# DigITs-AIML/MMNN_STS

Measured on AMD Instinct MI355X. Metric: training volumes/sec/GPU (128^3 T1+T2+preop, batch 2) at 1/2/4/8 MI355X, higher is better.
Workload: dtype f32; 1 GPU; configs[2] --images --preop --survival --blend: MultiModalModel(DenseNet121-3D(in=2), MLP(32), blend) fwd + GradientBlender Cox loss + bwd + grad all-reduce + SGD-Nesterov/OneCycle step, dropout 0.2; micro_batch=2, global_batch=2, tabular=32, parallelism=dp1, allreduce=none

## Files before the change

mmnn_sts_amd/csrc/densenet.hip:

```cpp
#include "densenet.hpp"

#include <string.h>

#include <algorithm>

#include "fprop.hpp"
#include "stem.hpp"
#include "wgrad.hpp"

namespace mmnn {

constexpr size_t KZ_PART_BYTES = (size_t)512 * 4 * 1024 * sizeof(float);
constexpr unsigned KZ_CNT_ENTRIES = 4096;

namespace {
struct Panel { const float* p; unsigned bytes; };
struct LayerBind {
  BnFwd bn1, bn2;
  BnBwd gr_new, gr_t1;
  StatPtr dg1, dg2, s_x;
  View x, g;
  View x_new, g_new;
  View t1, dz2;
};
// ... 361 lines not shown
      p.timer_ev.push_back(a); p.timer_ev.push_back(b);
      p.timer_tag.push_back(0);
    }
    p.timer_tag[p.timer_used / 2] = kind * MAX_BLOCKS + (block >= 0 && block < MAX_BLOCKS ? block : 0);
    on = hipEventRecord(p.timer_ev[p.timer_used], s) == hipSuccess;
  }
  ~ScopedTimer() {
    if (!on) return;
    (void)hipEventRecord(p.timer_ev[p.timer_used + 1], s);
    p.timer_used += 2;
  }
};
}

int plan_set_timer(Plan& p, int kind, int block) {
  MMNN_REQUIRE(kind >= -1 && kind < T_COUNT, "set_timer: unknown kernel class %d", kind);
  p.timer_mask = kind < 0 ? ~1u : (kind == T_NONE ? 0u : 1u << kind);
  p.timer_block = block; p.timer_used = 0;
  for (int k = 0; k < T_COUNT * MAX_BLOCKS; ++k) { p.timer_ms[k] = 0.0; p.timer_count[k] = 0; }
  return 0;
}

int plan_read_timer(Plan& p, int kind, int block, double* total_ms, long* count) {
  MMNN_REQUIRE(kind >= T_NONE && kind < T_COUNT && block < MAX_BLOCKS, "read_timer: unknown kernel class %d / block %d", kind, block);
  for (size_t i = 0; i + 1 < p.timer_used; i += 2) {
    MMNN_HIP(hipEventSynchronize(p.timer_ev[i + 1]));
    float ms = 0.f;
    MMNN_HIP(hipEventElapsedTime(&ms, p.timer_ev[i], p.timer_ev[i + 1]));
    const int k = p.timer_tag[i / 2];
    p.timer_ms[k] += ms; p.timer_count[k] += 1;
  }
  p.timer_used = 0;
  double ms = 0.0; long n = 0;
  for (int k = 1; k < T_COUNT; ++k)
    for (int b = 0; b < MAX_BLOCKS; ++b)
      if ((kind == T_NONE || kind == k) && (block < 0 || block == b)) { ms += p.timer_ms[k * MAX_BLOCKS + b]; n += p.timer_count[k * MAX_BLOCKS + b]; }
  if (total_ms) *total_ms = ms;
  if (count) *count = n;
  return 0;
}

int plan_set_option(Plan& p, const char* name, long value) {
  const std::string s(name ? name : "");
  if (s == "single_stream") return 0;
  if (s == "trace_buffer") { p.trace_base = reinterpret_cast<unsigned long long*>(value); p.trace_seq = 0; return 0; }
  if (s == "trace_slots") { p.trace_slots = (int)value; return 0; }
  if (s == "params_version") { p.params_version = value; return 0; }
  if (s == "no_kz") { p.no_kz = value != 0; return 0; }
  if (s == "conv1_dgrad_resident") {
    MMNN_REQUIRE(value >= 0 && value <= 2, "set_option: conv1_dgrad_resident is 0, 1 or 2");
    p.conv1_dgrad_resident = (int)value;
    return 0;
  }
  set_error("set_option: unknown option '%s'", s.c_str());
  return 1;
}
static DropCfg dropcfg(const Plan& p, uint64_t seed, int layer, int training) {
  DropCfg d; memset(&d, 0, sizeof(d));
  d.seed = seed; d.layer = layer; d.p = training ? p.cfg.dropout_p : 0.f;
  return d;
}

int plan_forward(Plan& p, const float* params, float* run, const float* x, char* ws, float* out, int training, uint64_t seed,
                 hipStream_t stream) {
  MMNN_REQUIRE(params && run && x && ws && out, "forward: null buffer");
  MMNN_REQUIRE(((uintptr_t)ws & 255) == 0 && ((uintptr_t)params & 15) == 0 && ((uintptr_t)x & 15) == 0, "forward: buffers must be 256/16-byte aligned");
  const NetCfg& c = p.cfg;
  const int nb = c.nblocks, N = p.N;
  if (!p.host_jobs) {
    MMNN_HIP(hipHostMalloc(&p.host_jobs, p.host_jobs_bytes, hipHostMallocDefault));
    memset(p.host_jobs, 0, p.host_jobs_bytes);
  }
  if (p.tab_params != params || p.tab_run != run || p.tab_ws != ws) {
    if (p.tab_ws != nullptr) MMNN_HIP(hipStreamSynchronize(stream));
    build_tables(p, params, run, ws);
    MMNN_HIP(hipMemcpyAsync(ws + p.o_jobs_run, p.host_jobs, p.host_jobs_bytes, hipMemcpyHostToDevice, stream));
  }
  p.trace_seq = 0;
  if (training) MMNN_HIP(hipMemsetAsync(ws + p.o_fstat, 0, p.fstat_bytes, stream));
  MMNN_HIP(hipMemsetAsync(ws + p.o_kz_cnt, 0, KZ_CNT_ENTRIES * sizeof(unsigned), stream));
  int rc = 0;
  if (p.params_version == 0 || p.params_version != p.packed_version || p.packed_params != params || p.packed_ws != ws) {
    rc = launch_pack(reinterpret_cast<const PackJob*>(ws + p.o_jobs_pack), p.n_pack_jobs, p.max_pack, stream);
    if (rc) return rc;
    p.packed_version = p.params_version; p.packed_params = params; p.packed_ws = ws;
    ++p.pack_launches;
  }

  {
    const NormSite n0 = norm0(p);
    StemConvArgs a; memset(&a, 0, sizeof(a));
    a.N = N; a.Cin = c.in_channels; a.D = p.D; a.H = p.H; a.W = p.W; a.Do = p.D0; a.Ho = p.H0; a.Wo = p.W0; a.M = c.init_features;
    a.x = x; a.wp = fptr(ws, p.o_pk_conv0); a.out = fptr(ws, p.o_conv0);
    a.st_out = stats(ws, n0, 0, training);
    { ScopedTimer t(p, T_STEM_CONV, -1, stream); rc = launch_stem_conv(a, stream); }
    if (rc) return rc;
    const View X = concat(p, ws, 0);
    StemPoolArgs q; memset(&q, 0, sizeof(q));
    q.N = N; q.C = c.init_features; q.Di = p.D0; q.Hi = p.H0; q.Wi = p.W0; q.Do = p.Db[0]; q.Ho = p.Hb[0]; q.Wo = p.Wb[0];
    q.x = fptr(ws, p.o_conv0);
    q.bn = bnfwd(p, ws, params, run, n0, training);
    q.out = X.p; q.out_ns = X.ns;
    q.idx = reinterpret_cast<unsigned char*>(ws + p.o_idx);
    q.st_out = stats(ws, norm1(p, 0, 0), 0, training);
    if ((rc = launch_stem_pool(q, stream))) return rc;
  }
// ... 33 lines not shown
      q.bn = bnfwd(p, ws, params, run, tr, training);
      q.out = pooled(p, ws, b).p;
      if ((rc = launch_bnrelu_avgpool(q, stream))) return rc;
      FpropArgs a = block_args(p, ws, b + 1);
      a.Cin = p.trans[b].cin; a.M = p.trans[b].cout;
      set_in0(a, pooled(p, ws, b));
      a.w = trans_panel(p, ws, b).p; a.w_ld = a.M;
      set_out(a, concat(p, ws, b + 1));
      a.st_out = stats(ws, norm1(p, b + 1, 0), 0, training);
      prefetch(a, conv1_panel(p, ws, b + 1, 0));
      if ((rc = launch_fprop(a, 1, PRO_NONE, EPI_STORE_STATS, stream))) return rc;
    } else {
      const NormSite n5 = norm5(p);
      BnApplyArgs q; memset(&q, 0, sizeof(q));
      q.N = N; q.C = n5.C; q.V = p.Vb[b];
      q.x = X.p; q.x_ns = X.ns;
      q.bn = bnfwd(p, ws, params, run, n5, training);
      q.out = out;
      if ((rc = launch_bn_apply(q, stream))) return rc;
    }
  }
  if (training) {
    if ((rc = launch_running_stats(reinterpret_cast<const RunStatJob*>(ws + p.o_jobs_run), p.n_run_jobs, c.momentum,
                                   p.nbt_count == p.n_run_jobs ? p.nbt : nullptr, stream))) return rc;
  }
  return 0;
}

static LayerBind layer_bind(const Plan& p, const float* params, float* run, char* ws, int b, int l) {
  const NormSite n1 = norm1(p, b, l), n2 = norm2(p, b, l);
  LayerBind L; memset(&L, 0, sizeof(L));
  L.bn1 = bnfwd(p, ws, params, run, n1, 1); L.bn2 = bnfwd(p, ws, params, run, n2, 1);
  L.gr_new = bnbwd(p, ws, params, n1, n1.C); L.gr_t1 = bnbwd(p, ws, params, n2);
  L.dg1 = dgsums(ws, n1); L.dg2 = dgsums(ws, n2); L.s_x = sums(ws, n1);
  L.x = concat(p, ws, b); L.g = concat_grad(p, ws, b);
  L.x_new = concat(p, ws, b, n1.C); L.g_new = concat_grad(p, ws, b, n1.C);
  L.t1 = t1(p, ws, b, l); L.dz2 = dz2(p, ws, b, l);
  return L;
}

static void layer_wgrad_args(const Plan& p, const LayerBind& L, char* ws, int b, int l, int layer_id, WgradArgs& w2, WgradArgs& w1) {
  const int cin = p.layers[b][l].cin;
  wgrad_shape(w2, p, b);
  w2.M = p.cfg.growth; w2.Cin = p.mid;
  set_g0(w2, L.g_new); set_g1(w2, L.x_new); w2.gr = L.gr_new;
  w2.drop.layer = layer_id; w2.drop.p = p.cfg.dropout_p;
  set_x(w2, L.t1); w2.bn = L.bn2;
  w2.slab = fptr(ws, p.o_sl_c2[b][l]); w2.slab_stride = conv2_elems(p); w2.nsplit = p.ns_c2[b][l];
  wgrad_shape(w1, p, b);
  w1.M = p.mid; w1.Cin = cin;
  set_g0(w1, L.dz2); set_g1(w1, L.t1); w1.gr = L.gr_t1;
  set_x(w1, L.x); w1.bn = L.bn1;
  w1.slab = fptr(ws, p.o_sl_c1[b][l]); w1.slab_stride = conv1_elems(p, cin); w1.nsplit = p.ns_c1[b][l];
}

static ConsumerBwdArgs consumer_bwd_args(const Plan& p, const float* params, float* run, char* ws, const NormSite& s, int b, int mode, const float* dy) {
  const View X = concat(p, ws, b), G = concat_grad(p, ws, b);
  const StatPtr dg = dgsums(ws, s);
  ConsumerBwdArgs a; memset(&a, 0, sizeof(a));
  a.N = p.N; a.C = s.C; a.D = p.Db[b]; a.H = p.Hb[b]; a.W = p.Wb[b]; a.mode = mode; a.nrep = s.nrep;
  a.dy = dy; a.x = X.p; a.x_ns = X.ns;
  a.bn = bnfwd(p, ws, params, run, s, 1);
  a.g = G.p; a.g_ns = G.ns; a.dbeta = dg.sum; a.dgamma = dg.sq;
  a.s_acc = sums(ws, s);
  return a;
}

int plan_backward(Plan& p, const float* params, const float* x, char* ws, const float* grad_out, float* grad_params, int accumulate,
                  uint64_t seed, hipStream_t stream) {
  return plan_backward_range(p, params, x, ws, grad_out, grad_params, accumulate, seed, p.cfg.nblocks - 1, 0, stream);
}

int plan_block_param_range(const Plan& p, int block, long* begin, long* end) {
  const int nb = p.cfg.nblocks;
  MMNN_REQUIRE(block >= -1 && block < nb && begin && end, "block_param_range: block %d out of range [-1, %d)", block, nb);
  if (block < 0) { *begin = 0; *end = norm1(p, 0, 0).w; return 0; }
  *begin = norm1(p, block, 0).w;
  *end = (block + 1 < nb) ? norm1(p, block + 1, 0).w : p.n_params;
  return 0;
}

int plan_backward_range(Plan& p, const float* params, const float* x, char* ws, const float* grad_out, float* grad_params, int accumulate,
                        uint64_t seed, int hi, int lo, hipStream_t stream) {
  MMNN_REQUIRE(params && x && ws && grad_out && grad_params, "backward: null buffer");
  MMNN_REQUIRE(p.tab_ws == ws && p.tab_params == params, "backward: must follow a training forward on the same buffers");
  const NetCfg& c = p.cfg;
  const int nb = c.nblocks, N = p.N;
  MMNN_REQUIRE(hi >= lo && lo >= 0 && hi < nb, "backward: bad block range [%d, %d] of %d blocks", lo, hi, nb);
  MMNN_REQUIRE(hi == nb - 1 || p.bwd_next == hi, "backward: block range [%d, %d] out of order (expected to continue at block %d)", lo, hi, p.bwd_next);
  float* run = p.tab_run;
  int rc;
  const bool first_call = hi == nb - 1;
  if (first_call) {
    MMNN_HIP(hipMemsetAsync(ws + p.o_bstat, 0, p.bstat_bytes, stream));
    MMNN_HIP(hipMemsetAsync(ws + p.o_kz_cnt, 0, KZ_CNT_ENTRIES * sizeof(unsigned), stream));
  }
  p.bwd_next = lo - 1;
  if (first_call || !p.wg_uploaded) {
    const size_t bytes = sizeof(WgradArgs) * 2 * p.n_layers;
    if (!p.wg_pinned) {
      MMNN_HIP(hipHostMalloc(&p.wg_pinned, bytes, hipHostMallocDefault));
      p.wg_shadow.assign(bytes, 0);
      p.wg_uploaded = false;
    }
    std::vector<WgradArgs> tab(2 * p.n_layers);
    int id = 0;
// ... 24 lines not shown
      int i = j - 1;
      while (i > id0 && wgrad1_channel_width(host_w1[i - 1].Cin, p.Vb[b]) == wgrad1_channel_width(host_w1[j - 1].Cin, p.Vb[b])) --i;
      {
        ScopedTimer t(p, T_CONV1_WGRAD, b, stream);
        rc2 = j - i > 1 ? launch_wgrad_batched(host_w1 + i, dev_w1 + i, j - i, seed, 1, PRO_BNRELU, stream)
                        : launch_wgrad1(host_w1[i], PRO_BNRELU, stream);
      }
      if (rc2) return rc2;
      j = i;
    }
    return 0;
  };
  if (first_call && (rc = launch_consumer_bwd(consumer_bwd_args(p, params, run, ws, norm5(p), nb - 1, 0, grad_out), stream))) return rc;
  int layer_id = 0;
  for (int b = 0; b <= hi; ++b) layer_id += c.block_layers[b];
  for (int b = hi; b >= lo; --b) {
    for (int l = c.block_layers[b] - 1; l >= 0; --l) {
      --layer_id;
      const LayerBind L = layer_bind(p, params, run, ws, b, l);
      const int cin = p.layers[b][l].cin;
      FpropArgs a = block_args(p, ws, b);
      a.Cin = c.growth; a.M = p.mid;
      set_in0(a, L.g_new); set_in1(a, L.x_new); a.gr_in = L.gr_new;
      a.drop_in = dropcfg(p, seed, layer_id, 1);
      set_conv2_weights(a, p, ws, b, l, true); a.w_ld = p.mid;
      set_out(a, L.dz2); set_ex(a, L.t1); a.ebn = L.bn2;
      a.dbeta = L.dg2.sum; a.dgamma = L.dg2.sq;
      prefetch(a, conv1_weights(p, params, b, l));
      { ScopedTimer t(p, T_CONV2_DGRAD, b, stream); rc = launch_fprop(a, 27, PRO_GRAD, EPI_MASK_STORE, stream); }
      if (rc) return rc;
      FpropArgs d = block_args(p, ws, b);
      d.Cin = p.mid; d.M = cin;
      set_in0(d, L.dz2); set_in1(d, L.t1); d.gr_in = L.gr_t1;
      d.w = conv1_weights(p, params, b, l).p; d.w_ld = cin;
      set_out(d, L.g); set_ex(d, L.x); d.ebn = L.bn1;
      d.dbeta = L.dg1.sum; d.dgamma = L.dg1.sq;
      d.s_acc = L.s_x;
      if (l > 0) prefetch(d, conv2_panel(p, ws, b, l - 1, true));
      { ScopedTimer t(p, T_CONV1_DGRAD, b, stream); rc = launch_fprop(d, 1, PRO_GRAD, EPI_MASK_ACCUM, stream); }
      if (rc) return rc;
    }
    if ((rc = block_wgrads(b, layer_id))) return rc;
    const View X = concat(p, ws, b), G = concat_grad(p, ws, b);
    const BnBwd gr = bnbwd(p, ws, params, norm1(p, b, 0));
    if (b > 0) {
      const int pb = b - 1;
      const TransOff& t = p.trans[pb];
      WgradArgs w;
      wgrad_shape(w, p, b);
      w.M = t.cout; w.Cin = t.cin;
      set_g0(w, G); set_g1(w, X); w.gr = gr;
      set_x(w, pooled(p, ws, pb));
      w.slab = fptr(ws, p.o_sl_tr[pb]); w.slab_stride = trans_elems(t); w.nsplit = p.ns_tr[pb];
      if ((rc = launch_wgrad1(w, PRO_NONE, stream))) return rc;
      FpropArgs d = block_args(p, ws, b);
      d.nrep = 0;
      d.Cin = t.cout; d.M = t.cin;
      set_in0(d, G); set_in1(d, X); d.gr_in = gr;
      d.w = params + t.cw; d.w_ld = t.cin;
      set_out(d, pooled_grad(p, ws, pb));
      if ((rc = launch_fprop(d, 1, PRO_GRAD, EPI_STORE, stream))) return rc;
      if ((rc = launch_consumer_bwd(consumer_bwd_args(p, params, run, ws, transition(p, pb), pb, 1, pooled_grad(p, ws, pb).p), stream))) return rc;
    } else {
      const NormSite n0 = norm0(p);
      const StatPtr dg = dgsums(ws, n0);
      StemPoolBwdArgs q; memset(&q, 0, sizeof(q));
      q.N = N; q.C = c.init_features; q.Di = p.D0; q.Hi = p.H0; q.Wi = p.W0; q.Do = p.Db[0]; q.Ho = p.Hb[0]; q.Wo = p.Wb[0];
      q.x = fptr(ws, p.o_conv0);
      q.bn = bnfwd(p, ws, params, run, n0, 1);
      q.g = G.p; q.g_ns = G.ns; q.xp = X.p; q.xp_ns = X.ns;
      q.gr = gr;
      q.idx = reinterpret_cast<const unsigned char*>(ws + p.o_idx);
      q.dz = fptr(ws, p.o_dz0);
      q.dbeta = dg.sum; q.dgamma = dg.sq;
      if ((rc = launch_stem_pool_bwd(q, stream))) return rc;
      StemWgradArgs w; memset(&w, 0, sizeof(w));
      w.N = N; w.Cin = c.in_channels; w.D = p.D; w.H = p.H; w.W = p.W; w.Do = p.D0; w.Ho = p.H0; w.Wo = p.W0; w.M = c.init_features;
      w.x = x; w.dz = fptr(ws, p.o_dz0); w.y = fptr(ws, p.o_conv0);
      w.gr = bnbwd(p, ws, params, n0);
      w.slab = fptr(ws, p.o_sl_conv0); w.slab_stride = (long)c.in_channels * c.init_features * 352; w.nsplit = p.ns_conv0;
      { ScopedTimer t(p, T_STEM_WGRAD, -1, stream); rc = launch_stem_wgrad(w, stream); }
      if (rc) return rc;
    }
  }
  const long stem_count = (long)c.init_features * c.in_channels * 343;
  const GradJob* jobs = reinterpret_cast<const GradJob*>(ws + p.o_jobs_grad);
  const int j0 = lo == 0 ? 0 : p.gj_begin[lo], j1 = p.gj_begin[hi + 1];
  long jmax = lo == 0 ? stem_count : 0;
  for (int b = lo; b <= hi; ++b) jmax = std::max(jmax, p.gj_max[b]);
  return launch_finalize(jobs + j0, j1 - j0, jmax, grad_params, accumulate, stream);
}

int plan_relu_mask(Plan& p, const float* params, char* ws, int kind, int b, int l, unsigned char* out, hipStream_t stream) {
  MMNN_REQUIRE(p.tab_ws == ws && p.tab_params == params, "relu_mask: must follow a training forward on the same buffers");
  const NetCfg& c = p.cfg;
  MMNN_REQUIRE(kind == 0 || (b >= 0 && b < c.nblocks), "relu_mask: bad block %d", b);
  MMNN_REQUIRE(kind != 3 || b < c.nblocks - 1, "relu_mask: block %d has no transition", b);
  MMNN_REQUIRE(kind == 0 || kind == 3 || (l >= 0 && l < c.block_layers[b] && (kind == 1 || kind == 2)), "relu_mask: bad site (%d,%d,%d)", kind, b, l);
  const NormSite s = kind == 0 ? norm0(p) : kind == 1 ? norm1(p, b, l) : kind == 2 ? norm2(p, b, l) : transition(p, b);
  const int V = kind == 0 ? p.D0 * p.H0 * p.W0 : p.Vb[b];
  const View X = kind == 0 ? View{fptr(ws, p.o_conv0), (long)s.C * V, 0} : kind == 2 ? t1(p, ws, b, l) : concat(p, ws, b);
  MaskArgs a; memset(&a, 0, sizeof(a));
  a.out = out; a.N = p.N; a.C = s.C; a.V = V; a.x = X.p; a.x_ns = X.ns;
  a.bn = bnfwd(p, ws, params, p.tab_run, s, 1);
  return launch_relu_mask(a, stream);
}
// ... 41 lines not shown
```

mmnn_sts_amd/csrc/densenet.hpp:

```cpp
#pragma once
#include <string>
#include <vector>

#include "common.hpp"
#include "elementwise.hpp"

namespace mmnn {

constexpr int MAX_BLOCKS = 8;

struct NetCfg {
  int in_channels, init_features, growth, bn_size, nblocks;
  int block_layers[MAX_BLOCKS];
  float eps, momentum, dropout_p;
};

struct LayerOff {
  long n1w, n1b, c1, n2w, n2b, c2;
  long r1m, r1v, r2m, r2v;
  int cin;
};
struct TransOff { long nw, nb, cw; long rm, rv; int cin, cout; };

struct NormSite {
// ... 7 lines not shown
struct View { float* p; long ns; int coff; };

struct Plan {
  NetCfg cfg;
  int N, D, H, W;
  int D0, H0, W0;
  int Db[MAX_BLOCKS], Hb[MAX_BLOCKS], Wb[MAX_BLOCKS], Vb[MAX_BLOCKS];
  int cin_b[MAX_BLOCKS], ctot_b[MAX_BLOCKS];
  int nrep_b[MAX_BLOCKS];
  int mid;
  long p_conv0, p_n0w, p_n0b, r_n0m, r_n0v, p_n5w, p_n5b, r_n5m, r_n5v;
  std::vector<std::vector<LayerOff>> layers;
  std::vector<TransOff> trans;
  long n_params, n_runstats;
  int n_bn;
  size_t ws_bytes;
  size_t o_conv0, o_idx, o_x[MAX_BLOCKS], o_g[MAX_BLOCKS], o_ap[MAX_BLOCKS], o_dz2[MAX_BLOCKS], o_dap, o_dz0;
  std::vector<std::vector<size_t>> o_t1;
  size_t o_fstat, fstat_bytes, o_bstat, bstat_bytes;
  size_t o_st_conv0, o_st_x[MAX_BLOCKS];
  std::vector<std::vector<size_t>> o_st_t1;
  size_t o_s_x[MAX_BLOCKS];
  size_t o_dg_n0, o_dg_n5;
  std::vector<std::vector<size_t>> o_dg_n1, o_dg_n2;
  std::vector<size_t> o_dg_tr;
  size_t o_pk_conv0;
  std::vector<std::vector<size_t>> o_pk_c1, o_pk_c2f, o_pk_c2b;
  std::vector<std::vector<size_t>> o_pk_c2f3, o_pk_c2b3;
  size_t o_x3 = 0, x3_bytes = 0;
  std::vector<size_t> o_pk_tr;
  size_t o_sl_conv0; int ns_conv0;
  std::vector<std::vector<size_t>> o_sl_c1, o_sl_c2;
  std::vector<std::vector<int>> ns_c1, ns_c2;
  std::vector<size_t> o_sl_tr; std::vector<int> ns_tr;
  size_t o_kz_part, o_kz_cnt;
  size_t o_jobs_run, o_jobs_pack, o_jobs_grad;
  int n_layers = 0;
  size_t o_wg_table = 0;
  void* wg_pinned = nullptr; std::vector<char> wg_shadow; bool wg_uploaded = false;
  void* host_jobs = nullptr; size_t host_jobs_bytes = 0;
  const float* tab_params = nullptr; float* tab_run = nullptr; char* tab_ws = nullptr;
  int n_run_jobs = 0, n_pack_jobs = 0, n_grad_jobs = 0; long max_pack = 0, max_grad = 0;
  int gj_begin[MAX_BLOCKS + 1] = {0};
  long gj_max[MAX_BLOCKS] = {0};
  unsigned timer_mask = 0; int timer_block = -1;
  std::vector<hipEvent_t> timer_ev;
  std::vector<int> timer_tag;
  size_t timer_used = 0;
  double timer_ms[16 * MAX_BLOCKS] = {0}; long timer_count[16 * MAX_BLOCKS] = {0};
  long params_version = 0, packed_version = 0; const float* packed_params = nullptr; const char* packed_ws = nullptr;
  long pack_launches = 0;
  long long* nbt = nullptr; int nbt_count = 0;
  int conv1_dgrad_resident = 1;
  bool no_kz = false;
  int bwd_next = -1;
  unsigned long long* trace_base = nullptr; mutable int trace_seq = 0; int trace_slots = 0;
};

enum TimerKind { T_NONE = 0, T_CONV2_FWD = 1, T_CONV2_DGRAD = 2, T_CONV2_WGRAD = 3, T_CONV1_FWD = 4, T_CONV1_DGRAD = 5,
                 T_CONV1_WGRAD = 6, T_STEM_CONV = 7, T_STEM_WGRAD = 8, T_BLOCK_FWD = 9, T_COUNT = 10 };
int plan_set_timer(Plan& p, int kind, int block);
int plan_read_timer(Plan& p, int kind, int block, double* total_ms, long* count);
int plan_set_option(Plan& p, const char* name, long value);

int plan_build(Plan& p, const NetCfg& cfg, int N, int D, int H, int W);
void plan_free(Plan& p);
int plan_forward(Plan& p, const float* params, float* runstats, const float* x, char* ws, float* out, int training,
                 uint64_t seed, hipStream_t stream);
int plan_backward(Plan& p, const float* params, const float* x, char* ws, const float* grad_out, float* grad_params,
                  int accumulate, uint64_t seed, hipStream_t stream);
int plan_backward_range(Plan& p, const float* params, const float* x, char* ws, const float* grad_out, float* grad_params,
                        int accumulate, uint64_t seed, int hi, int lo, hipStream_t stream);
int plan_block_param_range(const Plan& p, int block, long* begin, long* end);
long plan_ws_offset(const Plan& p, const char* name, int i, int j);
int plan_relu_mask(Plan& p, const float* params, char* ws, int kind, int b, int l, unsigned char* out, hipStream_t stream);

}
```

mmnn_sts_amd/csrc/wgrad.hip:

```cpp
#include "wgrad.hpp"

#include <algorithm>

namespace mmnn {

static void wg3_tile(int W, int& TD, int& TH, int& TW) {
  if (W > 16) { TD = 1; TH = 2; TW = 32; }
  else if (W > 8) { TD = 1; TH = 4; TW = 16; }
  else if (W > 4) { TD = 2; TH = 4; TW = 8; }
  else { TD = 4; TH = 4; TW = 4; }
}

static int wg1_wc(int Cin, long V) {
  const int thr = V >= 32768 ? 256 : 97;
  return Cin >= thr ? 8 : 4;
}

int wgrad_pick_splits(int taps, int N, int D, int H, int W, int M, int Cin, int batch) {
  if (batch < 1) batch = 1;
  if (taps == 27) {
    int TD, TH, TW;
    wg3_tile(W, TD, TH, TW);
    const long ntiles = (long)N * cdiv(D, TD) * cdiv(H, TH) * cdiv(W, TW);
    const int cgroups = cdiv(Cin, 32);
    long s = 512 / ((long)cgroups * batch);
    if (s > 64) s = 64;
    if (s > ntiles / 2) s = ntiles / 2;
    return s < 1 ? 1 : (int)s;
  }
  const long V = (long)D * H * W;
  const long nchunks = (long)N * cdiv(V, 64);
  const int wc = wg1_wc(Cin, V);
  constexpr long target = 2048;
  const long groups = (long)cdiv(Cin, 32 * wc) * cdiv(M, 128);
  long s = batch > 1 ? target / batch : target / groups;
  const long slab_cap = ((long)64 << 20) / ((long)M * Cin * 4);
  if (s > slab_cap) s = slab_cap;
  if (s > nchunks / 2) s = nchunks / 2;
  return s < 1 ? 1 : (int)s;
}

int wgrad1_channel_width(int Cin, long V) { return 32 * wg1_wc(Cin, V); }

int wgrad3_launch_batched(const WgradArgs* host, const WgradArgs* dev, int count, uint64_t seed, hipStream_t stream);
int wgrad1_launch(const WgradArgs& a, int pro_x, int wc, hipStream_t s);
int wgrad1_launch_batched(const WgradArgs* host, const WgradArgs* dev, int count, uint64_t seed, int wc, hipStream_t stream);

int launch_wgrad_batched(const WgradArgs* host, const WgradArgs* dev, int count, uint64_t seed, int taps, int pro_x, hipStream_t stream) {
  MMNN_REQUIRE(host && dev && count >= 1 && count <= 65535, "wgrad batch: bad table (count %d)", count);
  MMNN_REQUIRE(pro_x == PRO_BNRELU, "wgrad batch: only the dense-layer kernels (BN+ReLU input prologue) are batched");
  MMNN_REQUIRE(taps == 1 || taps == 27, "wgrad: taps must be 1 or 27");
  const WgradArgs& f = host[0];
  for (int i = 0; i < count; ++i) {
    const WgradArgs& a = host[i];
    MMNN_REQUIRE(a.N == f.N && a.D == f.D && a.H == f.H && a.W == f.W && a.M == f.M, "wgrad batch: layer %d differs in extent", i);
    MMNN_REQUIRE(a.N > 0 && a.D > 0 && a.H > 0 && a.W > 0 && a.Cin > 0 && a.M > 0, "wgrad: non-positive extent");
    MMNN_REQUIRE((long)a.D * a.H * a.W < (1l << 30), "wgrad: volume too large for 32-bit voxel indices");
    MMNN_REQUIRE(taps != 27 || (long)33 * a.D * a.H * a.W < (1l << 31), "wgrad: volume too large for 32-bit element offsets of a 32-channel group");
    MMNN_REQUIRE(a.g0 && a.g1 && a.x && a.slab, "wgrad: null operand");
    MMNN_REQUIRE(a.nsplit >= 1 && a.nsplit <= 65535, "wgrad: bad split count %d", a.nsplit);
    MMNN_REQUIRE(a.slab_stride >= (long)taps * a.M * a.Cin, "wgrad: slab stride too small");
    MMNN_REQUIRE(taps == 27 ? a.M <= 32 : a.M <= 128, "wgrad batch: %d output channels exceed one block row", a.M);
    MMNN_REQUIRE(taps == 27 || wg1_wc(a.Cin, (long)a.D * a.H * a.W) == wg1_wc(f.Cin, (long)f.D * f.H * f.W), "wgrad batch: layer %d needs another channel-group width", i);
  }
  if (taps == 27) return wgrad3_launch_batched(host, dev, count, seed, stream);
  return wgrad1_launch_batched(host, dev, count, seed, wg1_wc(f.Cin, (long)f.D * f.H * f.W), stream);
}

int launch_wgrad1(const WgradArgs& a, int pro_x, hipStream_t stream) {
  MMNN_REQUIRE(a.N > 0 && a.D > 0 && a.H > 0 && a.W > 0 && a.Cin > 0 && a.M > 0, "wgrad: non-positive extent");
  MMNN_REQUIRE((long)a.D * a.H * a.W < (1l << 30), "wgrad: volume too large for 32-bit voxel indices");
  MMNN_REQUIRE(a.g0 && a.g1 && a.x && a.slab, "wgrad: null operand");
  MMNN_REQUIRE(a.nsplit >= 1 && a.nsplit <= 65535, "wgrad: bad split count %d", a.nsplit);
  MMNN_REQUIRE(a.slab_stride >= (long)a.M * a.Cin, "wgrad: slab stride too small");
  MMNN_REQUIRE(pro_x == PRO_BNRELU || pro_x == PRO_NONE, "wgrad: unsupported input prologue %d", pro_x);
  return wgrad1_launch(a, pro_x, wg1_wc(a.Cin, (long)a.D * a.H * a.W), stream);
}

}
```

mmnn_sts_amd/csrc/wgrad.hpp:

```cpp
#pragma once
#include <type_traits>

#include "common.hpp"
#include "wgrad_tile.hpp"

namespace mmnn {

struct WgradArgs {
  int N, D, H, W;
  int M, Cin;
  const float* g0; long g0_ns; int g0_coff;
  const float* g1; long g1_ns; int g1_coff;
  BnBwd gr;
  DropCfg drop;
  const float* x; long x_ns; int x_coff;
  BnFwd bn;
  float* slab; long slab_stride; int nsplit;
  unsigned long long* trace;
};

int launch_wgrad1(const WgradArgs& a, int pro_x, hipStream_t stream);
int launch_wgrad_batched(const WgradArgs* host, const WgradArgs* dev_table, int count, uint64_t seed, int taps, int pro_x, hipStream_t stream);
int wgrad1_channel_width(int Cin, long V);
int wgrad_pick_splits(int taps, int N, int D, int H, int W, int M, int Cin, int batch = 1);

#if defined(__HIPCC__)

#if !defined(MMNN_TRACE_TID)
#define MMNN_TRACE_TID 0
#endif

template <int TD, int TH, int TW>
struct Wg3Cfg {
  static constexpr int VT = TD * TH * TW;
  static constexpr int RS = TW + 2, HS = TH + 2, DS = TD + 2;
  static constexpr int XS = (DS * HS * RS) | 1;
  static constexpr int YS = VT + 1;
  static constexpr int NTHREADS = 8 * 64;
  static_assert(VT == 64, "tile must hold 64 voxels (two per MFMA k-step, 32 steps)");
  static_assert(32 % TW == 0, "tile width must divide 32");
  static constexpr int STAGE = 32 * XS + 32 * YS;
  static size_t smem_bytes() { return sizeof(float) * (2 * STAGE + 3 * 32 + 2 * 32 + 3 * 32); }
};

template <int NTP, int TD, int TH, int TW, class F>
__device__ __forceinline__ void wg3_mfma(f32x16 (&acc)[4], const float* yl, const float* x0, const float* x1, const float* x2, const float* x3, F&& filler) {
  constexpr int RS = Wg3Cfg<TD, TH, TW>::RS, HS = Wg3Cfg<TD, TH, TW>::HS;
  mfma_ksteps<32, 1, NTP>(
      acc, [&](int s, float (&av)[1]) { av[0] = yl[s]; },
      [&](int s, float (&bv)[NTP]) {
        int wx, hy, dz;
        tile_local<TH, TW>(s, wx, hy, dz);
        const int p0 = (dz * HS + hy) * RS + wx;
        bv[0] = x0[p0]; bv[1] = x1[p0]; bv[2] = x2[p0];
        if constexpr (NTP == 4) bv[3] = x3[p0];
      },
      filler);
}

template <int PRO_X, int TD, int TH, int TW>
__device__ __forceinline__ void wgrad3_body(const WgradArgs& a, const int split, const int cg) {
  using C = Wg3Cfg<TD, TH, TW>;
  constexpr int RS = C::RS, HS = C::HS, DS = C::DS, XS = C::XS, YS = C::YS, NTHREADS = C::NTHREADS;
  extern __shared__ __attribute__((aligned(16))) float smem[];
  float* Xs = smem;
  float* Ys = Xs + 32 * XS;
  float* gcoef = smem + 2 * C::STAGE;
  float* xcoef = gcoef + 96;
  float* gbase = xcoef + 64;
  const int tid = threadIdx.x, lane = tid & 63, wave = tid >> 6, half = lane >> 5, l31 = lane & 31;
// ... 216 lines not shown
      const int d = d0 + dz - 1, h = h0 + hy - 1, w = w0 + q - 1;
      const bool ok = c0 + cl < a.Cin && (unsigned)d < (unsigned)a.D && (unsigned)h < (unsigned)a.H && (unsigned)w < (unsigned)a.W;
      const float x = xn[ok ? (long)cl * V + ((long)d * a.H + h) * a.W + w : 0];
      Xs[cl * XS + (dz * HS + hy) * RS + q] = ok ? pro_apply<PRO_X>(xcoef, 32, cl, x, 0.f) : 0.f;
    }
#pragma unroll 4
    for (int it = tid; it < 32 * 64; it += NTHREADS) {
      const int t = it & 63, m = it >> 6;
      int wx, hy, dz;
      tile_local<TH, TW>(t, wx, hy, dz);
      const int d = d0 + dz, h = h0 + hy, w = w0 + wx;
      const bool ok = m < a.M && d < a.D && h < a.H && w < a.W;
      const long g = ok ? (long)m * V + ((long)d * a.H + h) * a.W + w : 0;
      const float o = pro_apply<PRO_GRAD>(gcoef, 32, m, g0n[g], g1n[g]);
      Ys[m * YS + t] = ok ? o : 0.f;
    }
    __syncthreads();
    mfma_tile(0, NoFiller{});
    __syncthreads();
  }
  }
  float* out = a.slab + (long)split * a.slab_stride + c0 + l31;
#pragma unroll
  for (int j = 0; j < 4; ++j)
    if (j < ntap) store_acc_tile(acc[j], out + (long)(tap0 + j) * a.M * a.Cin, a.Cin, 0, a.M, half, c0 + l31 < a.Cin);
}

template <int PRO_X, int TD, int TH, int TW>
__global__ void __launch_bounds__(512) wgrad3_batched_kernel(const WgradArgs* __restrict__ table, const uint64_t seed, const int nsplit,
                                                             const int cgroups, const int ngroups) {
  int z, split, cg;
  if (ngroups > 0) {
    const int lin = blockIdx.x, x = lin & 7, j = lin >> 3;
    const int G = x + 8 * (j / cgroups);
    cg = j % cgroups;
    if (G >= ngroups) return;
    z = G / nsplit; split = G - z * nsplit;
  } else {
    z = blockIdx.z; split = blockIdx.x; cg = blockIdx.y;
  }
  WgradArgs a = table[z];
  if (split >= a.nsplit || cg * 32 >= a.Cin) return;
  a.drop.seed = seed;
  wgrad3_body<PRO_X, TD, TH, TW>(a, split, cg);
}

template <int WC>
struct Wg1Cfg {
  static constexpr int VK = 64, S = VK + 1;
  static constexpr int NTHREADS = WC * 64;
  static size_t smem_bytes() { return sizeof(float) * (128 * S + 32 * WC * S + 3 * 128 + 2 * 32 * WC + 3 * 128); }
};

template <int PRO_X, int WC>
__device__ __forceinline__ void wgrad1_body(const WgradArgs& a, const int split, const int c0, const int m0) {
  using C = Wg1Cfg<WC>;
  constexpr int S = C::S, VK = C::VK, NTHREADS = C::NTHREADS, CB = 32 * WC;
  extern __shared__ __attribute__((aligned(16))) float smem[];
  float* As = smem;
  float* Bs = As + 128 * S;
  float* gcoef = Bs + CB * S;
  float* xcoef = gcoef + 384;
  float* gbase = xcoef + 2 * CB;
  const int tid = threadIdx.x, lane = tid & 63, wave = tid >> 6, half = lane >> 5, l31 = lane & 31;
  const int V = a.D * a.H * a.W;
  const int chunks_per_n = (V + VK - 1) / VK;
  int k_begin, k_end;
  split_range(a.N * chunks_per_n, split, a.nsplit, k_begin, k_end);

  auto coefficients = [&]() {
    for (int c = tid; c < CB; c += NTHREADS) pro_coef_row(xcoef, CB, c, c0 + c, PRO_X == PRO_BNRELU && c0 + c < a.Cin, a.bn);
    for (int m = tid; m < 128; m += NTHREADS) pro_coef_row(gbase, 128, m, m0 + m, m0 + m < a.M, a.gr);
  };
  f32x16 acc[4] = {};
  const float* al = As + l31 * S + 32 * half;
  const float* bl = Bs + (wave * 32 + l31) * S + 32 * half;
  const bool wave_has_channels = c0 + wave * 32 < a.Cin;
  const bool vec = (V & 3) == 0 && ((((uintptr_t)a.x | (uintptr_t)a.g0 | (uintptr_t)a.g1) & 15) == 0);

  auto mfma_chunk = [&]() {
    mfma_ksteps<32, 4, 1>(
        acc,
        [&](int s, float (&av)[4]) {
#pragma unroll
          for (int t = 0; t < 4; ++t) av[t] = al[t * 32 * S + s];
        },
        [&](int s, float (&bv)[1]) { bv[0] = bl[s]; }, NoFiller{});
  };

  if (vec) {
    constexpr int A_ITEMS = 128 * (VK / 4), B_ITEMS = CB * (VK / 4);
    constexpr int A_IT = (A_ITEMS + NTHREADS - 1) / NTHREADS, B_IT = (B_ITEMS + NTHREADS - 1) / NTHREADS;
    f32x4 ga[A_IT], gb[A_IT], xb[B_IT];
    unsigned oka = 0, okb = 0;
    auto load_chunk = [&](int ch) {
      const int n = ch / chunks_per_n, v0 = (ch % chunks_per_n) * VK;
      const gcf xn = (gcf)a.x + (long)n * a.x_ns + (long)(a.x_coff + c0) * V;
      const gcf g0n = (gcf)a.g0 + (long)n * a.g0_ns + (long)(a.g0_coff + m0) * V;
      const gcf g1n = (gcf)a.g1 + (long)n * a.g1_ns + (long)(a.g1_coff + m0) * V;
      oka = okb = 0;
#pragma unroll
      for (int i = 0; i < A_IT; ++i) {
        const int it = tid + i * NTHREADS;
        const int q = it % (VK / 4), m = it / (VK / 4);
        const int v = v0 + 4 * q;
        const bool ok = (it < A_ITEMS) && m0 + m < a.M && v < V;
        const long go = ok ? (long)m * V + v : 0;
        oka |= (ok ? 1u : 0u) << i;
        ga[i] = *reinterpret_cast<const MMNN_GLOBAL f32x4*>(g0n + go);
        gb[i] = *reinterpret_cast<const MMNN_GLOBAL f32x4*>(g1n + go);
      }
#pragma unroll
      for (int i = 0; i < B_IT; ++i) {
        const int it = tid + i * NTHREADS;
        const int q = it % (VK / 4), c = it / (VK / 4);
        const int v = v0 + 4 * q;
        const bool ok = (it < B_ITEMS) && c0 + c < a.Cin && v < V;
        okb |= (ok ? 1u : 0u) << i;
        xb[i] = *reinterpret_cast<const MMNN_GLOBAL f32x4*>(xn + (ok ? (long)c * V + v : 0));
      }
    };
    auto store_chunk = [&]() {
#pragma unroll
      for (int i = 0; i < A_IT; ++i) {
        const int it = tid + i * NTHREADS;
        if (it < A_ITEMS) {
          const int q = it % (VK / 4), m = it / (VK / 4);
          const bool ok = (oka >> i) & 1u;
#pragma unroll
          for (int e = 0; e < 4; ++e) As[m * S + 4 * q + e] = ok ? pro_apply<PRO_GRAD>(gcoef, 128, m, ga[i][e], gb[i][e]) : 0.f;
        }
      }
#pragma unroll
      for (int i = 0; i < B_IT; ++i) {
        const int it = tid + i * NTHREADS;
        if (it < B_ITEMS) {
          const int q = it % (VK / 4), c = it / (VK / 4);
          const bool ok = (okb >> i) & 1u;
#pragma unroll
          for (int e = 0; e < 4; ++e) Bs[c * S + 4 * q + e] = ok ? pro_apply<PRO_X>(xcoef, CB, c, xb[i][e], 0.f) : 0.f;
        }
      }
    };
// ... 13 lines not shown
      pt.lap(1);
      __syncthreads();
      pt.lap(2);
      if (ch + 1 < k_end) load_chunk(ch + 1);
      pt.lap(3);
      if (wave_has_channels) mfma_chunk();
      pt.lap(4);
      __syncthreads();
      pt.lap(5);
    }
    pt.finish(a.trace, split, 1, a.M, a.Cin, k_end - k_begin);
  } else {
  coefficients();
  int cur_n = -1;
  for (int ch = k_begin; ch < k_end; ++ch) {
    const int n = ch / chunks_per_n;
    const int v0 = (ch % chunks_per_n) * VK;
    if (n != cur_n) {
      __syncthreads();
      rescale_rows(gbase, gcoef, 128, m0, n, a.drop, tid, NTHREADS);
      cur_n = n;
      __syncthreads();
    }
    const float* xn = a.x + (long)n * a.x_ns + (long)(a.x_coff + c0) * V;
    const float* g0n = a.g0 + (long)n * a.g0_ns + (long)(a.g0_coff + m0) * V;
    const float* g1n = a.g1 + (long)n * a.g1_ns + (long)(a.g1_coff + m0) * V;
#pragma unroll 2
    for (int it = tid; it < 128 * VK; it += NTHREADS) {
      const int q = it % VK, m = it / VK;
      const int v = v0 + q;
      float o = 0.f;
      if (m0 + m < a.M && v < V) o = pro_apply<PRO_GRAD>(gcoef, 128, m, g0n[(long)m * V + v], g1n[(long)m * V + v]);
      As[m * S + q] = o;
    }
#pragma unroll 2
    for (int it = tid; it < CB * VK; it += NTHREADS) {
      const int q = it % VK, c = it / VK;
      const int v = v0 + q;
      float o = 0.f;
      if (c0 + c < a.Cin && v < V) o = pro_apply<PRO_X>(xcoef, CB, c, xn[(long)c * V + v], 0.f);
      Bs[c * S + q] = o;
    }
    __syncthreads();
    if (wave_has_channels) mfma_chunk();
    __syncthreads();
  }
  }
  const int c = c0 + wave * 32 + l31;
  float* out = a.slab + (long)split * a.slab_stride + c;
#pragma unroll
  for (int t = 0; t < 4; ++t) store_acc_tile(acc[t], out, a.Cin, m0 + t * 32, a.M, half, c < a.Cin);
}

template <int PRO_X, int WC>
__global__ void __launch_bounds__(WC * 64) wgrad1_kernel(const WgradArgs a) {
  wgrad1_body<PRO_X, WC>(a, blockIdx.x, blockIdx.y * (32 * WC), blockIdx.z * 128);
}

template <int PRO_X, int WC>
__global__ void __launch_bounds__(WC * 64) wgrad1_batched_kernel(const WgradArgs* __restrict__ table, const uint64_t seed) {
  const int split = blockIdx.x, cg = blockIdx.y;
  WgradArgs a = table[blockIdx.z];
  if (split >= a.nsplit || cg * (32 * WC) >= a.Cin) return;
  a.drop.seed = seed;
  wgrad1_body<PRO_X, WC>(a, split, cg * (32 * WC), 0);
}

#endif
}
```

mmnn_sts_amd/csrc/wgrad_k1.hip:

```cpp
#include <algorithm>

#include "wgrad.hpp"

namespace mmnn {

template <int PRO_X, int WC>
static int launch1(const WgradArgs& a, hipStream_t stream) {
  using C = Wg1Cfg<WC>;
  constexpr auto kern = wgrad1_kernel<PRO_X, WC>;
  const size_t smem = C::smem_bytes();
  if (int rc = allow_dynamic_lds<kern>(smem)) return rc;
  MMNN_LAUNCH(kern, dim3(a.nsplit, cdiv(a.Cin, 32 * WC), cdiv(a.M, 128)), dim3(C::NTHREADS), smem, stream, a);
  MMNN_HIP(hipGetLastError());
  return 0;
}

template <int PRO_X, int WC>
static int launch1_batched(const WgradArgs* host, const WgradArgs* dev, int count, uint64_t seed, hipStream_t stream) {
  using C = Wg1Cfg<WC>;
  constexpr auto kern = wgrad1_batched_kernel<PRO_X, WC>;
  const size_t smem = C::smem_bytes();
  if (int rc = allow_dynamic_lds<kern>(smem)) return rc;
  int gx = 1, gy = 1;
  for (int i = 0; i < count; ++i) { gx = std::max(gx, host[i].nsplit); gy = std::max(gy, cdiv(host[i].Cin, 32 * WC)); }
  MMNN_LAUNCH(kern, dim3(gx, gy, count), dim3(C::NTHREADS), smem, stream, dev, seed);
  MMNN_HIP(hipGetLastError());
  return 0;
}

int wgrad1_launch(const WgradArgs& a, int pro_x, int wc, hipStream_t s) {
  if (pro_x == PRO_BNRELU) return wc == 8 ? launch1<PRO_BNRELU, 8>(a, s) : launch1<PRO_BNRELU, 4>(a, s);
  return wc == 8 ? launch1<PRO_NONE, 8>(a, s) : launch1<PRO_NONE, 4>(a, s);
}

int wgrad1_launch_batched(const WgradArgs* host, const WgradArgs* dev, int count, uint64_t seed, int wc, hipStream_t stream) {
  return wc == 8 ? launch1_batched<PRO_BNRELU, 8>(host, dev, count, seed, stream) : launch1_batched<PRO_BNRELU, 4>(host, dev, count, seed, stream);
}

}
```

Baseline: 264.8 volumes/s (whole job; 1 volume = 1 patient = stacked T1+T2 2x128^3 + 32 tabular).

## Software-pipeline the 1x1 wgrad tile loop, interleaving global loads with MFMA k-steps

Adds a pipelined variant of the 1x1 weight-gradient kernel that splits each 32-wide chunk into two 16-step halves. It issues the global loads and LDS stores for the next half inside the MFMA k-steps using sched_group_barrier, and precomputes per-row prologue coefficients into registers. It also sets launch bounds to allow two blocks per CU for the pipelined kernel and turns it on by default behind a new option. The aim is to hide global-memory latency behind the matrix math, at the cost of more registers and more complex scheduling.

New measurement: 266.3 volumes/s (whole job; 1 volume = 1 patient = stacked T1+T2 2x128^3 + 32 tabular), median of 6. Within noise of the previous version (+0.6%).

```diff
diff --git a/mmnn_sts_amd/csrc/densenet.hip b/mmnn_sts_amd/csrc/densenet.hip
--- a/mmnn_sts_amd/csrc/densenet.hip
+++ b/mmnn_sts_amd/csrc/densenet.hip
@@ -437,6 +437,11 @@
     p.conv1_dgrad_resident = (int)value;
     return 0;
   }
+  if (s == "wgrad1_pipelined") {
+    MMNN_REQUIRE(value == 0 || value == 1, "set_option: wgrad1_pipelined is 0 or 1");
+    p.wgrad1_pipelined = (int)value;
+    return 0;
+  }
   set_error("set_option: unknown option '%s'", s.c_str());
   return 1;
 }
@@ -576,6 +581,7 @@
   set_g0(w1, L.dz2); set_g1(w1, L.t1); w1.gr = L.gr_t1;
   set_x(w1, L.x); w1.bn = L.bn1;
   w1.slab = fptr(ws, p.o_sl_c1[b][l]); w1.slab_stride = conv1_elems(p, cin); w1.nsplit = p.ns_c1[b][l];
+  w1.pipelined = p.wgrad1_pipelined;
 }
 
 static ConsumerBwdArgs consumer_bwd_args(const Plan& p, const float* params, float* run, char* ws, const NormSite& s, int b, int mode, const float* dy) {
@@ -706,6 +712,7 @@
       set_g0(w, G); set_g1(w, X); w.gr = gr;
       set_x(w, pooled(p, ws, pb));
       w.slab = fptr(ws, p.o_sl_tr[pb]); w.slab_stride = trans_elems(t); w.nsplit = p.ns_tr[pb];
+      w.pipelined = p.wgrad1_pipelined;
       if ((rc = launch_wgrad1(w, PRO_NONE, stream))) return rc;
       FpropArgs d = block_args(p, ws, b);
       d.nrep = 0;
diff --git a/mmnn_sts_amd/csrc/densenet.hpp b/mmnn_sts_amd/csrc/densenet.hpp
--- a/mmnn_sts_amd/csrc/densenet.hpp
+++ b/mmnn_sts_amd/csrc/densenet.hpp
@@ -83,6 +83,7 @@
   long pack_launches = 0;
   long long* nbt = nullptr; int nbt_count = 0;
   int conv1_dgrad_resident = 1;
+  int wgrad1_pipelined = 1;
   bool no_kz = false;
   int bwd_next = -1;
   unsigned long long* trace_base = nullptr; mutable int trace_seq = 0; int trace_slots = 0;
diff --git a/mmnn_sts_amd/csrc/wgrad.hip b/mmnn_sts_amd/csrc/wgrad.hip
--- a/mmnn_sts_amd/csrc/wgrad.hip
+++ b/mmnn_sts_amd/csrc/wgrad.hip
@@ -62,6 +62,7 @@
     MMNN_REQUIRE(a.slab_stride >= (long)taps * a.M * a.Cin, "wgrad: slab stride too small");
     MMNN_REQUIRE(taps == 27 ? a.M <= 32 : a.M <= 128, "wgrad batch: %d output channels exceed one block row", a.M);
     MMNN_REQUIRE(taps == 27 || wg1_wc(a.Cin, (long)a.D * a.H * a.W) == wg1_wc(f.Cin, (long)f.D * f.H * f.W), "wgrad batch: layer %d needs another channel-group width", i);
+    MMNN_REQUIRE(a.pipelined == f.pipelined, "wgrad batch: layer %d differs in the tile loop it asks for", i);
   }
   if (taps == 27) return wgrad3_launch_batched(host, dev, count, seed, stream);
   return wgrad1_launch_batched(host, dev, count, seed, wg1_wc(f.Cin, (long)f.D * f.H * f.W), stream);
diff --git a/mmnn_sts_amd/csrc/wgrad.hpp b/mmnn_sts_amd/csrc/wgrad.hpp
--- a/mmnn_sts_amd/csrc/wgrad.hpp
+++ b/mmnn_sts_amd/csrc/wgrad.hpp
@@ -16,6 +16,7 @@
   const float* x; long x_ns; int x_coff;
   BnFwd bn;
   float* slab; long slab_stride; int nsplit;
+  int pipelined;
   unsigned long long* trace;
 };
 
@@ -338,7 +339,7 @@
   static size_t smem_bytes() { return sizeof(float) * (128 * S + 32 * WC * S + 3 * 128 + 2 * 32 * WC + 3 * 128); }
 };
 
-template <int PRO_X, int WC>
+template <int PRO_X, int WC, bool PIPE>
 __device__ __forceinline__ void wgrad1_body(const WgradArgs& a, const int split, const int c0, const int m0) {
   using C = Wg1Cfg<WC>;
   constexpr int S = C::S, VK = C::VK, NTHREADS = C::NTHREADS, CB = 32 * WC;
@@ -374,7 +375,131 @@
         [&](int s, float (&bv)[1]) { bv[0] = bl[s]; }, NoFiller{});
   };
 
-  if (vec) {
+  if (vec && PIPE) {
+    constexpr int HQ = 8, RSTEP = NTHREADS / HQ;
+    constexpr int A_IT = 128 / RSTEP, B_IT = CB / RSTEP;
+    static_assert(128 % RSTEP == 0 && CB % RSTEP == 0, "rows must deal out evenly");
+    constexpr int SA = (A_IT + 1) / 2, SB = (B_IT + 1) / 2;
+    constexpr int LOAD_A = SA, STORE_B = SA + 1, LOAD_B = SA + 1 + SB;
+    static_assert(LOAD_B < 16, "staging pieces must fit the k-steps of a half");
+    const int r0 = tid / HQ, col = 4 * (tid & 3) + 32 * ((tid >> 2) & 1);
+    const long rowoff = (long)r0 * V + col, rstep = (long)RSTEP * V;
+    f32x4 ga[A_IT], gb[A_IT], xb[B_IT];
+    float gp[A_IT], gq[A_IT], gr[A_IT], xa[B_IT], xc[B_IT];
+    unsigned rowa = 0, rowb = 0;
+#pragma unroll
+    for (int i = 0; i < A_IT; ++i) rowa |= (m0 + r0 + i * RSTEP < a.M ? 1u : 0u) << i;
+#pragma unroll
+    for (int i = 0; i < B_IT; ++i) rowb |= (c0 + r0 + i * RSTEP < a.Cin ? 1u : 0u) << i;
+    bool cola = false, colb = false;
+    auto load_a = [&](int n, int v0) {
+      const gcf g0n = (gcf)a.g0 + (long)n * a.g0_ns + (long)(a.g0_coff + m0) * V;
+      const gcf g1n = (gcf)a.g1 + (long)n * a.g1_ns + (long)(a.g1_coff + m0) * V;
+      cola = v0 + col < V;
+#pragma unroll
+      for (int i = 0; i < A_IT; ++i) {
+        const long go = (cola && ((rowa >> i) & 1u)) ? rowoff + i * rstep + v0 : 0;
+        ga[i] = *reinterpret_cast<const MMNN_GLOBAL f32x4*>(g0n + go);
+        gb[i] = *reinterpret_cast<const MMNN_GLOBAL f32x4*>(g1n + go);
+      }
+    };
+    auto load_b = [&](int n, int v0) {
+      const gcf xn = (gcf)a.x + (long)n * a.x_ns + (long)(a.x_coff + c0) * V;
+      colb = v0 + col < V;
+#pragma unroll
+      for (int i = 0; i < B_IT; ++i)
+        xb[i] = *reinterpret_cast<const MMNN_GLOBAL f32x4*>(xn + ((colb && ((rowb >> i) & 1u)) ? rowoff + i * rstep + v0 : 0));
+    };
+    auto store_a = [&](int i, int hoff) {
+      const unsigned keep = (cola && ((rowa >> i) & 1u)) ? ~0u : 0u;
+      float* d = As + (r0 + i * RSTEP) * S + col + hoff;
+#pragma unroll
+      for (int e = 0; e < 4; ++e) d[e] = __uint_as_float(__float_as_uint(pro_elem<PRO_GRAD>(gp[i], gq[i], gr[i], ga[i][e], gb[i][e])) & keep);
+    };
+    auto store_b = [&](int i, int hoff) {
+      const unsigned keep = (colb && ((rowb >> i) & 1u)) ? ~0u : 0u;
+      float* d = Bs + (r0 + i * RSTEP) * S + col + hoff;
+#pragma unroll
+      for (int e = 0; e < 4; ++e) d[e] = __uint_as_float(__float_as_uint(pro_elem<PRO_X>(xa[i], xc[i], 0.f, xb[i][e], 0.f)) & keep);
+    };
+    auto stage = [&](int s, int hoff, int n, int v0) {
+#pragma unroll
+      for (int i = 0; i < A_IT; ++i)
+        if (i / 2 == s) store_a(i, hoff);
+      if (s == LOAD_A) { load_a(n, v0); __builtin_amdgcn_sched_group_barrier(0x020, 2 * A_IT, 0); }
+#pragma unroll
+      for (int i = 0; i < B_IT; ++i)
+        if (STORE_B + i / 2 == s) store_b(i, hoff);
+      if (s == LOAD_B) { load_b(n, v0); __builtin_amdgcn_sched_group_barrier(0x020, B_IT, 0); }
+    };
+    auto dout_coefficients = [&]() {
+#pragma unroll
+      for (int i = 0; i < A_IT; ++i) { const int m = r0 + i * RSTEP; gp[i] = gcoef[m]; gq[i] = gcoef[128 + m]; gr[i] = gcoef[256 + m]; }
+    };
+    auto run_half = [&](auto hoff_c, auto&& filler) {
+      constexpr int hoff = decltype(hoff_c)::value;
+      if (wave_has_channels) {
+        mfma_ksteps<16, 4, 1>(
+            acc,
+            [&](int s, float (&av)[4]) {
+#pragma unroll
+              for (int t = 0; t < 4; ++t) av[t] = al[t * 32 * S + hoff + s];
+            },
+            [&](int s, float (&bv)[1]) { bv[0] = bl[hoff + s]; }, filler);
+      } else {
+#pragma unroll
+        for (int s = 0; s < 16; ++s) filler(s);
+      }
+    };
+    using Half0 = std::integral_constant<int, 0>;
+    using Half1 = std::integral_constant<int, 16>;
+    PhaseTrace pt(a.trace != nullptr && tid == 0 && split < 16 && c0 == 0 && m0 == 0);
+    int n = k_begin / chunks_per_n, ci = k_begin % chunks_per_n;
+    int cur_n = n;
+    if (k_begin < k_end) { load_a(n, ci * VK); load_b(n, ci * VK); }
+    coefficients();
+    rescale_rows(gbase, gcoef, 128, m0, n, a.drop, tid, NTHREADS);
+    __syncthreads();
+    dout_coefficients();
+#pragma unroll
+    for (int i = 0; i < B_IT; ++i) { const int c = r0 + i * RSTEP; xa[i] = xcoef[c]; xc[i] = xcoef[CB + c]; }
+    if (k_begin < k_end) {
+#pragma unroll
+      for (int i = 0; i < A_IT; ++i) store_a(i, 0);
+#pragma unroll
+      for (int i = 0; i < B_IT; ++i) store_b(i, 0);
+      load_a(n, ci * VK + 16); load_b(n, ci * VK + 16);
+    }
+    __syncthreads();
+    pt.lap(0);
+    for (int ch = k_begin; ch < k_end; ++ch) {
+      const bool last = ch + 1 == k_end;
+      int n1 = n, c1 = ci;
+      if (!last && ++c1 == chunks_per_n) { c1 = 0; ++n1; }
+      const int v1 = c1 * VK;
+      run_half(Half0{}, [&](int s) { stage(s, 16, n1, v1); });
+      pt.lap(4);
+      __syncthreads();
+      pt.lap(5);
+      if (!last) {
+        if (n1 != cur_n) {
+          rescale_rows(gbase, gcoef, 128, m0, n1, a.drop, tid, NTHREADS);
+          cur_n = n1;
+          __syncthreads();
+          dout_coefficients();
+          pt.lap(1);
+        }
+        run_half(Half1{}, [&](int s) { stage(s, 0, n1, v1 + 16); });
+      } else {
+        run_half(Half1{}, NoFiller{});
+      }
+      pt.lap(4);
+      __syncthreads();
+      pt.lap(5);
+      n = n1; ci = c1;
+    }
+    pt.finish(a.trace, split, 1, a.M, a.Cin, k_end - k_begin);
+  } else if (vec) {
     constexpr int A_ITEMS = 128 * (VK / 4), B_ITEMS = CB * (VK / 4);
     constexpr int A_IT = (A_ITEMS + NTHREADS - 1) / NTHREADS, B_IT = (B_ITEMS + NTHREADS - 1) / NTHREADS;
     f32x4 ga[A_IT], gb[A_IT], xb[B_IT];
@@ -494,18 +619,18 @@
   for (int t = 0; t < 4; ++t) store_acc_tile(acc[t], out, a.Cin, m0 + t * 32, a.M, half, c < a.Cin);
 }
 
-template <int PRO_X, int WC>
-__global__ void __launch_bounds__(WC * 64) wgrad1_kernel(const WgradArgs a) {
-  wgrad1_body<PRO_X, WC>(a, blockIdx.x, blockIdx.y * (32 * WC), blockIdx.z * 128);
+template <int PRO_X, int WC, bool PIPE>
+__global__ void __launch_bounds__(WC * 64, PIPE ? 2 : 1) wgrad1_kernel(const WgradArgs a) {
+  wgrad1_body<PRO_X, WC, PIPE>(a, blockIdx.x, blockIdx.y * (32 * WC), blockIdx.z * 128);
 }
 
-template <int PRO_X, int WC>
-__global__ void __launch_bounds__(WC * 64) wgrad1_batched_kernel(const WgradArgs* __restrict__ table, const uint64_t seed) {
+template <int PRO_X, int WC, bool PIPE>
+__global__ void __launch_bounds__(WC * 64, PIPE ? 2 : 1) wgrad1_batched_kernel(const WgradArgs* __restrict__ table, const uint64_t seed) {
   const int split = blockIdx.x, cg = blockIdx.y;
   WgradArgs a = table[blockIdx.z];
   if (split >= a.nsplit || cg * (32 * WC) >= a.Cin) return;
   a.drop.seed = seed;
-  wgrad1_body<PRO_X, WC>(a, split, cg * (32 * WC), 0);
+  wgrad1_body<PRO_X, WC, PIPE>(a, split, cg * (32 * WC), 0);
 }
 
 #endif
diff --git a/mmnn_sts_amd/csrc/wgrad_k1.hip b/mmnn_sts_amd/csrc/wgrad_k1.hip
--- a/mmnn_sts_amd/csrc/wgrad_k1.hip
+++ b/mmnn_sts_amd/csrc/wgrad_k1.hip
@@ -4,10 +4,10 @@
 
 namespace mmnn {
 
-template <int PRO_X, int WC>
+template <int PRO_X, int WC, bool PIPE>
 static int launch1(const WgradArgs& a, hipStream_t stream) {
   using C = Wg1Cfg<WC>;
-  constexpr auto kern = wgrad1_kernel<PRO_X, WC>;
+  constexpr auto kern = wgrad1_kernel<PRO_X, WC, PIPE>;
   const size_t smem = C::smem_bytes();
   if (int rc = allow_dynamic_lds<kern>(smem)) return rc;
   MMNN_LAUNCH(kern, dim3(a.nsplit, cdiv(a.Cin, 32 * WC), cdiv(a.M, 128)), dim3(C::NTHREADS), smem, stream, a);
@@ -15,10 +15,10 @@
   return 0;
 }
 
-template <int PRO_X, int WC>
+template <int PRO_X, int WC, bool PIPE>
 static int launch1_batched(const WgradArgs* host, const WgradArgs* dev, int count, uint64_t seed, hipStream_t stream) {
   using C = Wg1Cfg<WC>;
-  constexpr auto kern = wgrad1_batched_kernel<PRO_X, WC>;
+  constexpr auto kern = wgrad1_batched_kernel<PRO_X, WC, PIPE>;
   const size_t smem = C::smem_bytes();
   if (int rc = allow_dynamic_lds<kern>(smem)) return rc;
   int gx = 1, gy = 1;
@@ -28,13 +28,20 @@
   return 0;
 }
 
+template <int PRO_X, int WC>
+static int launch1_loop(const WgradArgs& a, hipStream_t s) {
+  return a.pipelined ? launch1<PRO_X, WC, true>(a, s) : launch1<PRO_X, WC, false>(a, s);
+}
+
 int wgrad1_launch(const WgradArgs& a, int pro_x, int wc, hipStream_t s) {
-  if (pro_x == PRO_BNRELU) return wc == 8 ? launch1<PRO_BNRELU, 8>(a, s) : launch1<PRO_BNRELU, 4>(a, s);
-  return wc == 8 ? launch1<PRO_NONE, 8>(a, s) : launch1<PRO_NONE, 4>(a, s);
+  if (pro_x == PRO_BNRELU) return wc == 8 ? launch1_loop<PRO_BNRELU, 8>(a, s) : launch1_loop<PRO_BNRELU, 4>(a, s);
+  return wc == 8 ? launch1_loop<PRO_NONE, 8>(a, s) : launch1_loop<PRO_NONE, 4>(a, s);
 }
 
 int wgrad1_launch_batched(const WgradArgs* host, const WgradArgs* dev, int count, uint64_t seed, int wc, hipStream_t stream) {
-  return wc == 8 ? launch1_batched<PRO_BNRELU, 8>(host, dev, count, seed, stream) : launch1_batched<PRO_BNRELU, 4>(host, dev, count, seed, stream);
+  if (host[0].pipelined)
+    return wc == 8 ? launch1_batched<PRO_BNRELU, 8, true>(host, dev, count, seed, stream) : launch1_batched<PRO_BNRELU, 4, true>(host, dev, count, seed, stream);
+  return wc == 8 ? launch1_batched<PRO_BNRELU, 8, false>(host, dev, count, seed, stream) : launch1_batched<PRO_BNRELU, 4, false>(host, dev, count, seed, stream);
 }
 
 }
```
